# ChangwuLiu/InGVIO

Measured on AMD Instinct MI355X. Metric: ekf_updates_per_sec, higher is better.
Workload: dtype f64; 1 GPU; BASELINE configs[1]: synthetic stereo MSCKF, 150 feats x 11 clones, state dim N=249 (update at N), 512 independent filters per GPU; step = propagate(k=10)+clone+MSCKF update+marginalise; filters_per_gpu=512, feats=150, clones=11, state_dim=249, imu_steps=10, parallelism=independent filters, 1 rank(s), no data-path collective

## Files before the change

### include/ingvio_hip.h

```cpp
#ifndef INGVIO_HIP_H
#define INGVIO_HIP_H

#include <stddef.h>

#ifdef __cplusplus
extern "C" {
#endif

#define INGVIO_OK 0
#define INGVIO_NO_ROWS 1
#define INGVIO_NEG_DIAG 2
#define INGVIO_REJECTED 3
#define INGVIO_E_ARG (-1)
#define INGVIO_E_CAPACITY (-2)
#define INGVIO_E_HIP (-3)
#define INGVIO_E_NOT_IN_STATE (-4)
#define INGVIO_E_UNSUPPORTED (-5)
#define INGVIO_E_NOT_PD (-6)

typedef struct ingvio_ctx ingvio_ctx;

typedef struct {
    int batch;
    int n_max;
// ... 305 lines not shown
    int track;
    int anchor;
    double pf[3];
} ingvio_lm_init_cand;
typedef struct {
    int n_cand; const ingvio_lm_init_cand* cand;
    int n_drop; const int* drop_cols;
} ingvio_lm_init_block;
int ingvio_landmark_init_nominal(ingvio_ctx* ctx, int b0, int nb, const ingvio_lm_init_block* blocks, const ingvio_msckf_opts* opts,
                                 double chi2_mult, int do_chi2, int cand_cap,
                                 int* added, int* new_idx, int* slot, double* chi2, double* dx, int* status);
int ingvio_debug_landmark_init_rows(ingvio_ctx* ctx, int b, const ingvio_lm_init_cand* cand, const ingvio_msckf_opts* opts,
                                    int n_drop, const int* drop_cols, double* H_old, double* H_new, double* res, int* m_out);
int ingvio_frame_run(ingvio_ctx* ctx, int restore_prior);
int ingvio_set_frame_parts(ingvio_ctx* ctx, int parts);
int ingvio_frame_fetch(ingvio_ctx* ctx, int b0, int nb, double* dx_out, int* accepted, int* rows_out);
int ingvio_frame_fetch_begin(ingvio_ctx* ctx, int b0, int nb);
int ingvio_frame_fetch_end(ingvio_ctx* ctx, double* dx_out, int* accepted, int* rows_out);

int ingvio_debug_msckf_info(ingvio_ctx* ctx, int b, double* A_out, int* ncol_out);

int ingvio_debug_info_solution(ingvio_ctx* ctx, int b, double* out, int count);

int ingvio_debug_tracks_read(ingvio_ctx* ctx, int b, unsigned long long* mask, double* uv, double* pf);

int ingvio_debug_staged_frame(ingvio_ctx* ctx, int b, int* n_clones, int* n_feat, int* clone_idx, double* clone_R, double* clone_p,
                              int* anchor, int* dof, unsigned long long* obs_mask, double* pf, double* uv);

int ingvio_debug_read(ingvio_ctx* ctx, long long* out, int n);

// ... 10 lines not shown
```

### ingvio_amd/capi.py

```python
import ctypes as C
import os

import numpy as np

_HERE = os.path.dirname(os.path.abspath(__file__))
LIB_PATH = os.environ.get("INGVIO_HIP_LIB") or os.path.join(_HERE, "lib", "libingvio_hip.so")

c_dp = C.POINTER(C.c_double)
c_ip = C.POINTER(C.c_int)
c_up = C.POINTER(C.c_ulonglong)

OK, NO_ROWS, NEG_DIAG, REJECTED = 0, 1, 2, 3
E_ARG, E_CAPACITY, E_HIP, E_NOT_IN_STATE, E_UNSUPPORTED, E_NOT_PD = -1, -2, -3, -4, -5, -6
R_SCALAR, R_DIAG, R_FULL = 0, 1, 2

EXPORTS = [
    "ingvio_ctx_create", "ingvio_ctx_destroy", "ingvio_sync", "ingvio_ctx_stream", "ingvio_f_max", "ingvio_c_max", "ingvio_last_error", "ingvio_ldp",
    "ingvio_build_id",
    "ingvio_cov_set", "ingvio_cov_get", "ingvio_get_n", "ingvio_cov_get_marginal", "ingvio_cov_snapshot",
    "ingvio_cov_restore", "ingvio_propagate", "ingvio_propagate_fused", "ingvio_augment_clone", "ingvio_marginalize",
    "ingvio_append_independent", "ingvio_ekf_update", "ingvio_chi2_gamma", "ingvio_msckf_update", "ingvio_msckf_update_tri", "ingvio_qr_compress",
    "ingvio_frame_stage", "ingvio_frame_stage_async", "ingvio_frame_set_imu_noise", "ingvio_frame_fetch_begin", "ingvio_frame_fetch_end", "ingvio_tracks_create", "ingvio_frame_stage_tracks", "ingvio_frame_run", "ingvio_set_frame_parts", "ingvio_frame_fetch", "ingvio_profile_enable", "ingvio_profile_select",
    "ingvio_profile_reset",
    "ingvio_profile_get", "ingvio_set_msckf_method", "ingvio_set_qr_method", "ingvio_landmark_stage", "ingvio_landmark_run",
    "ingvio_landmark_fetch", "ingvio_frame_run_phase", "ingvio_info_set", "ingvio_debug_read", "ingvio_triangulate",
    "ingvio_gnss_front_stage", "ingvio_gnss_front_fetch", "ingvio_gnss_update_batch", "ingvio_gnss_stage", "ingvio_gnss_run", "ingvio_gnss_fetch", "ingvio_mld", "ingvio_debug_msckf_info", "ingvio_debug_info_solution",
    "ingvio_info_reduce", "ingvio_info_commit", "ingvio_gnss_sat_eval",
    "ingvio_chi2_gamma_multi", "ingvio_ekf_update_batch", "ingvio_add_variable_delayed_invertible", "ingvio_add_variable_delayed", "ingvio_add_variable_delayed_batch", "ingvio_replace_var_linear",
    "ingvio_nominal_create", "ingvio_nominal_set", "ingvio_nominal_get", "ingvio_nominal_box_plus", "ingvio_frame_stage_tracks_nominal",
    "ingvio_nominal_set_gnss", "ingvio_nominal_get_gnss", "ingvio_gnss_front_stage_nominal", "ingvio_landmark_stage_nominal",
    "ingvio_landmark_init_nominal", "ingvio_debug_landmark_init_rows", "ingvio_nominal_tail",
    "ingvio_debug_tracks_read", "ingvio_debug_staged_frame",
    "ingvio_gnss_frame_stage_nominal", "ingvio_debug_gnss_fused_last", "ingvio_debug_nominal_update_post",
]

NOM_NONE, NOM_SE23, NOM_SE3, NOM_VEC3, NOM_SCALAR, NOM_LANDMARK = -1, 0, 1, 2, 3, 4
NOM_VAL = 15
# ... 948 lines not shown
        fn = self.L.ingvio_frame_stage_async if use_async else self.L.ingvio_frame_stage

        def call(_keep=(keeps, chi2, sa, fa, o, sg)):
            self._chk(fn(self.h, b0, nb, sa, fa, C.byref(o), _d(sg), int(enable_gnss), C.c_double(sigma_cb), C.c_double(sigma_rw)))
        return call

    def frame_set_imu_noise(self, b0, noise):
        nz = f64(np.asarray(noise, dtype=np.float64).reshape(-1, 6))
        self._chk(self.L.ingvio_frame_set_imu_noise(self.h, int(b0), nz.shape[0], _d(nz)))

    def frame_run(self, restore_prior=False):
        self._chk(self.L.ingvio_frame_run(self.h, 1 if restore_prior else 0))

    def set_frame_parts(self, parts):
        self._chk(self.L.ingvio_set_frame_parts(self.h, int(parts)))

    def frame_fetch(self, b0=0, nb=None):
        nb = self.batch if nb is None else nb
        dx = np.zeros((nb, self.ldp)); acc = np.zeros((nb, self.f_max), dtype=np.int32); rows = np.zeros(nb, dtype=np.int32)
        self._chk(self.L.ingvio_frame_fetch(self.h, b0, nb, _d(dx), _i(acc), _i(rows)))
        return dx, acc, rows

    def frame_fetch_begin(self, b0=0, nb=None):
        nb = self.batch if nb is None else nb
        self._fetch_nb = nb
        self._chk(self.L.ingvio_frame_fetch_begin(self.h, b0, nb))

    def frame_fetch_end(self):
        nb = self._fetch_nb
        dx = np.empty((nb, self.ldp)); acc = np.empty((nb, self.f_max), dtype=np.int32); rows = np.empty(nb, dtype=np.int32)
# ... 85 lines not shown
```

### ingvio_amd/csrc/capi.hip

```cpp
#include "../../include/ingvio_hip.h"
#include "dev_common.h"
#include "launch_ekf.h"
#include "launch_msckf.h"
#include "launch_factored.h"
#include "launch_tri.h"
#include "launch_tracks.h"
#include "launch_lm.h"
#include "launch_delayed.h"
#include "launch_qr.h"
#include "launch_chol.h"
#include "launch_gnss.h"
#include "launch_lmbatch.h"
#include "launch_nominal.h"
#include "launch_tail.h"

#include <stdio.h>
#include <stdlib.h>
#include <string.h>
#include <unistd.h>
#include <string>
#include <atomic>
#include <cmath>
#include <condition_variable>
#include <functional>
// ... 125 lines not shown
    hipStream_t st2 = nullptr;
    hipEvent_t ev_fork = nullptr, ev_join = nullptr, ev_ref = nullptr;
    hipEvent_t ev_fetch = nullptr;
    int fetch_b0 = 0, fetch_nb = 0;
    hipStream_t st_copy = nullptr;
    hipEvent_t ev_copy = nullptr, ev_free[2] = { nullptr, nullptr };
    bool copy_pending = false, free_valid[2] = { false, false };
    int set_id = 0;
    struct PinSlab { char* p = nullptr; size_t cap = 0; hipEvent_t ev = nullptr; bool busy = false; };
    PinSlab pin[4];
    int pin_next = 0;
    struct PartStream { hipStream_t st = nullptr; hipEvent_t ev_gate = nullptr, ev_apply = nullptr, ev_done = nullptr; };
    PartStream part[4];
    int parts_alloc = 0;
    int parts_req = -1;
    bool split_pending = false;
    hipEvent_t tok_last = nullptr;
    hipEvent_t ev_split_fork = nullptr;
    hipStream_t run_st = nullptr;
    hipEvent_t tok_wait = nullptr, tok_rec = nullptr;
    struct Tracks { double *uv = nullptr, *pf = nullptr; unsigned long long* mask = nullptr; int t_max = 0; char* stage[2] = { nullptr, nullptr }; size_t stage_cap = 0; } trk;
    struct Nominal {
        int vmax = 0, ir = 0, dr = 0;
        int* ih = nullptr; double* dv = nullptr;
        int* ih_snap = nullptr; double* dv_snap = nullptr;
        double* dx = nullptr;
        std::vector<int> h_ih, h_ih_snap;
        bool has_snap = false;
        bool pending = false;
        bool frame = false;
// ... 555 lines not shown
    if (g.strong) { E.chi2 = g.chi2; E.chi2_len = g.chi2_len; E.gate_max_rows = 14; }
    RowsGateIn in{ g.H + (size_t)b0 * hs, g.res + (size_t)b0 * mld, g.noise + (size_t)b0 * mld, g.m + b0, g.colmap + (size_t)b0 * GNSS_NCW,
                   g.nc + b0, (int)hs, GNSS_NCW };
    {
        ProfScope p(c, PF_ROWGATE);
        if (launch_rows_gate(E, in, g.thr1, g.gamma + (size_t)b0 * mld, g.keep + (size_t)b0 * mld, c->run_st)) return INGVIO_E_CAPACITY;
    }
    { ProfScope p(c, PF_EKF_CORE); launch_ekf_core(E, c->run_st); }
    L.gY = E.Y; L.gYstride = ws; L.gm = g.mf + b0;
    g.fused_last = true; g.folded_last = true;
    g.results = true;
    return 0;
}

int run_msckf_factored(ingvio_ctx* c, int b0, int nb, const MsckfOpts& op, int stereo, int fmax_used,
                       const int* marg_idx = nullptr, int marg_size = 0, int phase = 0, bool gnss_fuse = false)
{
    FactoredLaunch L;
    memset(&L, 0, sizeof L);
    L.stereo = stereo; L.cv = view(c); L.fv = fview(c); L.op = op; L.b0 = b0; L.nb = nb;
    L.fmax_used = fmax_used > 0 ? fmax_used : 1;
    L.ncol_cap = 6 * c->d.c_max;
    for (int i = 0; i < nb; ++i) if (c->h_nclones[b0 + i] > L.c_used) L.c_used = c->h_nclones[b0 + i];
    L.gamma = c->d_gamma; L.accept = c->d_accept; L.used = c->d_used; L.rec = c->d_rec;
    L.Apart = c->d_Rpart + (size_t)b0 * c->G * c->rstride; L.chunk_used = c->d_chunk_used + (size_t)b0 * c->G;
    L.G = c->G; L.rstride = c->rstride; L.noise = c->d_noise + b0;
    L.Tflat = c->d_Tflat; L.tfstride = (size_t)c->ldp * 100; L.flat_nb = std::min(c->d.batch, APPLY_FLAT_NB);
    L.Asum = c->d_Asum ? c->d_Asum + (size_t)b0 * c->rstride : nullptr; L.used_sum = c->d_used_sum ? c->d_used_sum + b0 : nullptr;
#ifdef INGVIO_ALT_KERNELS
    static const bool few_off = [] { const char* e = getenv("INGVIO_FEW"); return e && !strcmp(e, "off"); }();
    if (few_off) { L.Tflat = nullptr; L.Asum = nullptr; }
// ... 16 lines not shown
    if (phase != 2) {
        if (c->tok_wait) HIPCHK(c, hipStreamWaitEvent(c->run_st, c->tok_wait, 0));
        {
            const bool pon = c->prof && (c->prof_only < 0 || c->prof_only == PF_GATE2);
            int used = 0;
            if (pon) { hipEventCreate(&L.prof_a); hipEventCreate(&L.prof_b); L.prof_used = &used; }
            L.stage = 0;
            const int grc = launch_factored(L, c->run_st);
            if (pon) {
                if (used) c->recs.push_back({ PF_GATE2, L.prof_a, L.prof_b });
                else { hipEventDestroy(L.prof_a); hipEventDestroy(L.prof_b); }
                L.prof_a = nullptr; L.prof_b = nullptr; L.prof_used = nullptr;
            }
            if (grc) return INGVIO_E_UNSUPPORTED;
        }
        { ProfScope p(c, PF_GRAM); L.stage = 1; launch_factored(L, c->run_st); }
        if (c->tok_rec) HIPCHK(c, hipEventRecord(c->tok_rec, c->run_st));
    }
    if (forked) {
        HIPCHK(c, hipStreamWaitEvent(c->st2, c->ev_fork, 0));
        L.stage = 6; launch_factored(L, c->st2);
        HIPCHK(c, hipEventRecord(c->ev_ref, c->st2));
        L.stage = 7; launch_factored(L, c->st2);
        HIPCHK(c, hipEventRecord(c->ev_join, c->st2));
    }
    if (phase == 1) return last_launch(c);
    if (forked) {
        ProfScope p(c, PF_INFO);
        HIPCHK(c, hipStreamWaitEvent(c->run_st, c->ev_ref, 0));
        L.stage = 8; launch_factored(L, c->run_st);
        HIPCHK(c, hipStreamWaitEvent(c->run_st, c->ev_join, 0));
        L.stage = 9; launch_factored(L, c->run_st);
    } else {
        if (big) { ProfScope p(c, PF_INFO); L.stage = 5; launch_factored(L, c->run_st); }
        { ProfScope p(c, PF_INFO); L.stage = 2; launch_factored(L, c->run_st); }
    }
    if (gnss_fuse) { if (int rc = gnss_in_frame_launch(c, b0, nb, L)) return rc; }
    if (phase == 2 && c->tok_wait) HIPCHK(c, hipStreamWaitEvent(c->run_st, c->tok_wait, 0));
    { ProfScope p(c, PF_APPLY); L.stage = 3; launch_factored(L, c->run_st); }
    if (phase == 2 && c->tok_rec) HIPCHK(c, hipEventRecord(c->tok_rec, c->run_st));
    return last_launch(c);
}

int run_msckf(ingvio_ctx* c, int b0, int nb, const MsckfOpts& op, int stereo, int fmax_used)
{
    if (c->method == 1) return run_msckf_factored(c, b0, nb, op, stereo, fmax_used);
    MsckfLaunch L;
    memset(&L, 0, sizeof L);
    L.stereo = stereo; L.cv = view(c); L.fv = fview(c); L.op = op; L.b0 = b0; L.nb = nb;
    L.fmax_used = fmax_used > 0 ? fmax_used : 1;
    L.gamma = c->d_gamma; L.accept = c->d_accept; L.used = c->d_used;
    L.Rpart = c->d_Rpart + (size_t)b0 * c->G * c->rstride; L.chunk_used = c->d_chunk_used + (size_t)b0 * c->G;
    L.G = c->G; L.rstride = c->rstride;
    L.Hout = c->d_H + (size_t)b0 * c->hstride; L.res_out = c->d_res + (size_t)b0 * c->mld;
    L.colmap = c->d_colmap + (size_t)b0 * c->cstride; L.m_out = c->d_m + b0; L.nc_out = c->d_nc + b0;
    L.mld = c->mld; L.hstride = c->hstride; L.cstride = c->cstride;
    { ProfScope p(c, PF_GATE); L.stage = 0; if (launch_msckf(L, c->st)) return INGVIO_E_UNSUPPORTED; }
    { ProfScope p(c, PF_FOLD); L.stage = 1; launch_msckf(L, c->st); }
    { ProfScope p(c, PF_MERGE); L.stage = 2; launch_msckf(L, c->st); }
    EkfLaunch E;
    memset(&E, 0, sizeof E);
// ... 135 lines not shown
    if (desc->c_max > bigwin_cmax()) return INGVIO_E_CAPACITY;
    if (desc->m_max > 128) return INGVIO_E_CAPACITY;
    int ndev = 0;
    if (hipGetDeviceCount(&ndev) != hipSuccess || ndev <= desc->device) return INGVIO_E_HIP;
    ingvio_ctx* c = new ingvio_ctx();
    c->d = *desc;
    if (c->d.m_max < 1) c->d.m_max = 32;
    c->err.clear();
    if (hipSetDevice(desc->device) != hipSuccess) { delete c; return INGVIO_E_HIP; }
    c->own_stream = desc->stream == nullptr;
    if (c->own_stream) {
        if (hipStreamCreateWithFlags(&c->st, hipStreamNonBlocking) != hipSuccess) { delete c; return INGVIO_E_HIP; }
    } else c->st = (hipStream_t)desc->stream;
    c->run_st = c->st;
    if (const char* e = getenv("INGVIO_FRAME_PARTS")) c->parts_req = atoi(e);
    if (desc->c_max > 16) {
        int lo = 0, hi = 0;
        hipDeviceGetStreamPriorityRange(&lo, &hi);
        if (hipStreamCreateWithPriority(&c->st2, hipStreamNonBlocking, hi) != hipSuccess) c->st2 = nullptr;
        if (c->st2 && (hipEventCreateWithFlags(&c->ev_fork, hipEventDisableTiming) != hipSuccess ||
                       hipEventCreateWithFlags(&c->ev_ref, hipEventDisableTiming) != hipSuccess ||
                       hipEventCreateWithFlags(&c->ev_join, hipEventDisableTiming) != hipSuccess)) { hipStreamDestroy(c->st2); c->st2 = nullptr; }
    }
    const int B = desc->batch;
    c->ldp = (desc->n_max + 15) & ~15;
    const int cls0 = desc->c_max > 16 ? bigwin_cmax() : msckf_cmax_class(desc->c_max);
    const int cpad = cls0 > desc->c_max ? cls0 : desc->c_max;
    const int mcap = c->d.m_max > 6 * cpad ? c->d.m_max : 6 * cpad;
    c->mld = (mcap + 15) & ~15;
    c->nc_cap = c->ldp > mcap ? c->ldp : mcap;
// ... 2859 lines not shown
    if (wait_inputs(c)) return INGVIO_E_HIP;
    launch_restore_propagate(c, restore_prior, strips_valid(c, restore_prior), 0, B, c->st);
    mirror_restore_clone(c, restore_prior);
    const bool with_lm = lm_in_frame(c);
    const bool fuse = c->method == 1 && !with_lm;
    const bool lm_oop = with_lm && c->method == 1;
    const bool gnss_here = gnss_in_frame(c), gnss_fuse = fuse && gnss_folds(c);
    const bool gnss_nomf = c->gn.staged && c->gn.frame_nom;
    if (gnss_nomf) {
        auto& g = c->gn;
        HIPCHK(c, hipMemsetAsync(g.dxf, 0, 8 * (size_t)B * c->ldp, c->st));
        HIPCHK(c, hipMemsetAsync(g.stf, 0, sizeof(int) * (size_t)B, c->st));
        HIPCHK(c, hipMemsetAsync(g.mf, 0, sizeof(int) * (size_t)B, c->st));
        g.own_status = true; g.results = true; g.fused_last = true; g.folded_last = false;
    }
    int rc = fuse     ? run_msckf_factored(c, 0, B, c->st_op, c->st_stereo, c->st_fmax_used, c->d_idx, 6, 0, gnss_fuse)
             : lm_oop ? run_msckf_factored(c, 0, B, c->st_op, c->st_stereo, c->st_fmax_used, c->d_zero_idx, 0)
                      : run_msckf(c, 0, B, c->st_op, c->st_stereo, c->st_fmax_used);
    if (rc) return rc;
    if (lm_oop) {
        if (!c->apply_flipped) launch_post_marg(view(c), 0, B, c->d_zero_idx, 0, c->st);
        for (int b = 0; b < B; ++b) c->h_cur[b] ^= 1;
    }
    const bool lm_nom = with_lm && c->lm.nominal;
    if (lm_nom) landmark_gather_launch(c, c->d_dx, 0, B);
    bool lm_fused = false;
    if (with_lm) { rc = landmark_update_launch(c, 0, B, c->d_idx, 6, &lm_fused); if (rc) return rc; }
    if (!(fuse && c->apply_flipped)) {
        ProfScope p(c, PF_MARG);
        if (fuse || lm_fused) launch_post_marg(view(c), 0, B, c->d_idx, 6, c->st);
        else launch_marginalize(view(c), 0, B, c->d.n_max, c->d_idx, 6, c->st);
    }
// ... 63 lines not shown
    const int P = std::min(c->parts_req > 0 ? c->parts_req : 1, 4);
    const bool gnss_fuse = gnss_folds(c);
    if (P > 1 && c->method == 1 && !lm_in_frame(c) && c->d.c_max <= 16 && (!gnss_in_frame(c) || gnss_fuse) && B >= 16 * P)
        return frame_run_split(c, restore_prior, P, gnss_fuse);
    return frame_run_whole(c, restore_prior);
}

int ingvio_frame_run(ingvio_ctx* c, int restore_prior) { return frame_run_impl(c, restore_prior, 0); }
int ingvio_set_frame_parts(ingvio_ctx* c, int parts)
{
    if (!c || parts < -1 || parts > 4) return INGVIO_E_ARG;
    ENTER(c);
    c->parts_req = parts == 0 ? 1 : parts;
    return INGVIO_OK;
}
int ingvio_frame_run_phase(ingvio_ctx* c, int restore_prior, int phase)
{
    if (phase < 0 || phase > 2) return INGVIO_E_ARG;
    return frame_run_impl(c, restore_prior, phase);
}

int ingvio_info_set(ingvio_ctx* c, int b, const double* A, int ncol, int n_accepted)
{
    ENTER(c);
    if (check_range(c, b, 1) || !A || ncol < 6 || (size_t)ncol * (ncol + 1) > (size_t)c->rstride || n_accepted < 0) return INGVIO_E_ARG;
    std::vector<int> used(c->G, 0);
    used[0] = n_accepted;
    int rc = up(c, c->d_Rpart + (size_t)b * c->G * c->rstride, A, 8 * (size_t)ncol * (ncol + 1));
    rc |= up(c, c->d_chunk_used + (size_t)b * c->G, used.data(), sizeof(int) * (size_t)c->G);
    if (rc) return INGVIO_E_HIP;
// ... 87 lines not shown
    return last_launch(c);
}

int ingvio_set_msckf_method(ingvio_ctx* c, int method)
{
    ENTER(c);
    if (!c || method < 0 || method > 1) return INGVIO_E_ARG;
    c->method = method;
    return INGVIO_OK;
}

int ingvio_debug_msckf_info(ingvio_ctx* c, int b, double* A_out, int* ncol_out)
{
    ENTER(c);
    if (check_range(c, b, 1) || !A_out || !ncol_out) return INGVIO_E_ARG;
    int C = 0;
    if (down_sync(c, &C, c->d_nclones + b, sizeof(int))) return INGVIO_E_HIP;
    const int ncol = 6 * C;
    *ncol_out = ncol;
    const size_t w = (size_t)ncol + 1;
    for (size_t e = 0; e < (size_t)ncol * w; ++e) A_out[e] = 0.0;
    if (c->method == 1) {
        std::vector<int> used(c->G);
        if (down_sync(c, used.data(), c->d_chunk_used + (size_t)b * c->G, sizeof(int) * (size_t)c->G)) return INGVIO_E_HIP;
        std::vector<double> part((size_t)ncol * w);
        for (int g = 0; g < c->G; ++g) {
            if (!used[g]) continue;
            if (down_sync(c, part.data(), c->d_Rpart + ((size_t)b * c->G + g) * c->rstride, 8 * part.size())) return INGVIO_E_HIP;
            for (size_t e = 0; e < part.size(); ++e) A_out[e] += part[e];
        }
// ... 139 lines not shown
```

### ingvio_amd/csrc/kernels_factored.hip

```cpp
#include <algorithm>
#include <stdlib.h>
#include <string.h>
#include "launch_factored.h"

#include "gate_kernel.h"
#include "gate5_kernel.h"
#include "gate5m_kernel.h"

#define GATE_FPW 1
template <int CMAX, bool STEREO>
__global__ __launch_bounds__(GATE_FPW * WAVE) __attribute__((amdgpu_waves_per_eu(2, 4))) void k_feat_gate3(
    CovView cv, FrameView fv, MsckfOpts op, int b0, int nb, int fmax_used, double* __restrict__ gamma_out,
    int* __restrict__ accept_out, double* __restrict__ rec_out)
{
    gate3_body<CMAX, STEREO, GATE_FPW, false>(cv, fv, op, b0, nb, fmax_used, gamma_out, accept_out, rec_out);
}

#ifndef GATE4_WPE
#define GATE4_WPE 2
#endif
#ifndef GATE4_WPE_MAX
#define GATE4_WPE_MAX 6
#endif
template <int CMAX>
// ... 21 lines not shown
}

#define GRAM_NB 8
#define GRAM_NT 256
#ifndef GRAM2_ZFORM
#define GRAM2_ZFORM 1
#endif
__device__ __forceinline__ double gram_rsqrt(double x)
{
    double y = __builtin_amdgcn_rsq(x);
    double e = fma(-x * y, y, 1.0);
    y = fma(y * e, fma(e, 0.375, 0.5), y);
    e = fma(-x * y, y, 1.0);
    return fma(y * e, 0.5, y);
}
template <int CMAX>
struct Gram2Cfg {
    static constexpr int NC = 6 * CMAX;
    static constexpr int TI = (NC + 15) / 16;
    static constexpr int TJ = (NC + 1 + 15) / 16;
    static constexpr int LDW = 16 * TJ;
    static constexpr int NTILE = TI * TJ;
    static constexpr int NUP = TI * TJ - TI * (TI - 1) / 2;
    static constexpr int TPW = (NUP + 3) / 4;
    static constexpr int KR = 3 * GRAM_NB;
    static constexpr int SPW = 34;
};
template <int CMAX>
struct Gram2Batch {
    using Cfg = Gram2Cfg<CMAX>;
    double Bm[Cfg::KR][Cfg::LDW];
    double Ym[Cfg::KR][Cfg::LDW];
    double sp[CMAX * CMAX <= 128 ? 2 : 1][GRAM_NB][CMAX][Cfg::SPW];
};
template <int CMAX>
struct Gram2Out {
    using Cfg = Gram2Cfg<CMAX>;
    double A2[Cfg::NC][Cfg::NC + 2];
    double S[CMAX][CMAX][34];
};

template <int CMAX, bool STEREO>
__global__ __launch_bounds__(GRAM_NT, 2) void k_feat_gram2(
    FrameView fv, MsckfOpts op, int b0, const int* __restrict__ accept_in, int* __restrict__ used_out,
    double* __restrict__ Apart, int* __restrict__ chunk_used, int G, int rstride)
{
    using Cfg = Gram2Cfg<CMAX>;
    constexpr int NC = Cfg::NC, TJ = Cfg::TJ, LDW = Cfg::LDW, NTILE = Cfg::NTILE, TPW = Cfg::TPW, KR = Cfg::KR;
    constexpr int NUP = Cfg::NUP, TI = Cfg::TI, RPO = STEREO ? 4 : 2;
    extern __shared__ __attribute__((aligned(16))) char smem_raw[];
    Gram2Batch<CMAX>& sb = *reinterpret_cast<Gram2Batch<CMAX>*>(smem_raw);
    Gram2Out<CMAX>& so = *reinterpret_cast<Gram2Out<CMAX>*>(smem_raw);
    constexpr size_t UNI = sizeof(Gram2Batch<CMAX>) > sizeof(Gram2Out<CMAX>) ? sizeof(Gram2Batch<CMAX>) : sizeof(Gram2Out<CMAX>);
    int* sUse = reinterpret_cast<int*>(smem_raw + ((UNI + 15) / 16) * 16);
    int* sList = sUse + fv.fmax;
    __shared__ int sNu;
    __shared__ double sPose[16][12];
    const int bl = blockIdx.y, b = b0 + bl, g = blockIdx.x, tid = threadIdx.x, lane = tid & 63, wave = __builtin_amdgcn_readfirstlane(tid >> 6);
    const int F = fv.n_feat[b], C = fv.n_clones[b], ncol = 6 * C;
    for (int e = tid; e < 12 * C; e += GRAM_NT) {
        const int c = e / 12, q = e - 12 * c;
        sPose[c][q] = q < 9 ? fv.clone_R[((size_t)b * fv.cmax + c) * 9 + q] : fv.clone_p[((size_t)b * fv.cmax + c) * 3 + q - 9];
    }

    dbg_stamp(32);
    for (int j = tid; j < F; j += GRAM_NT) {
        int use = accept_in[(size_t)b * fv.fmax + j];
        if (use && op.max_accept > 0) {
            int rank = 0;
            for (int q = 0; q < j; ++q) rank += accept_in[(size_t)b * fv.fmax + q];
            if (rank >= op.max_accept) use = 0;
        }
        sUse[j] = use;
        if (g == 0) used_out[(size_t)b * fv.fmax + j] = use;
    }
    for (int e = tid; e < KR * LDW; e += GRAM_NT) { (&sb.Bm[0][0])[e] = 0.0; (&sb.Ym[0][0])[e] = 0.0; }
    __syncthreads();
    if (wave == 0) {
        int cnt = 0;
        for (int base = 0; base < F; base += WAVE) {
            const int j = base + lane;
            const bool u = j < F && sUse[j];
            const unsigned long long m = __ballot(u);
            if (u) sList[cnt + __popcll(m & ((1ULL << lane) - 1ULL))] = j;
            cnt += __popcll(m);
        }
        if (lane == 0) sNu = cnt;
    }
    __syncthreads();
    const int nu = sNu, per = (nu + G - 1) / G;
    const int q0 = g * per, q1 = min(nu, q0 + per);

    dbg_stamp(33);
    int tiA[TPW], tjA[TPW];
#pragma unroll
    for (int u = 0; u < TPW; ++u) {
        int t = wave + 4 * u, ti = 0;
        while (ti < TI - 1 && t >= TJ - ti) { t -= TJ - ti; ++ti; }
        tiA[u] = ti; tjA[u] = ti + t;
    }
    double4_f acc[TPW];
#pragma unroll
    for (int u = 0; u < TPW; ++u) acc[u] = double4_f{ 0.0, 0.0, 0.0, 0.0 };
    constexpr bool OVL = CMAX * CMAX <= 128;
    const int ptid = OVL ? tid - 128 : tid;
    const int pc = ptid >= 0 ? ptid / CMAX : 0, pa = ptid >= 0 ? ptid - pc * CMAX : 0;
    const bool pairlane = ptid >= 0 && ptid < CMAX * CMAX;
    double sS1[9], sNX[9], sS3[9], s4[3], s5[3];
#pragma unroll
    for (int i = 0; i < 9; ++i) { sS1[i] = 0.0; sNX[i] = 0.0; sS3[i] = 0.0; }
#pragma unroll
    for (int i = 0; i < 3; ++i) { s4[i] = 0.0; s5[i] = 0.0; }
// ... 36 lines not shown
        }
    };
    auto sum16 = [](double v) {
#ifdef GRAM_SHFL_SUM
        v += __shfl_xor(v, 8, 16); v += __shfl_xor(v, 4, 16); v += __shfl_xor(v, 2, 16); v += __shfl_xor(v, 1, 16);
#else
        v += row_ror_f64<8>(v); v += row_ror_f64<4>(v); v += row_ror_f64<2>(v); v += row_ror_f64<1>(v);
#endif
        return v;
    };
    fetch(q0);
    auto do_p2 = [&](int qb, int buf, int nthr, bool rows, bool sparse) {
        const int nbf = min(GRAM_NB, q1 - qb);
        dbg_stamp(34);
        if (rows && nbf < GRAM_NB) {
            for (int e = tid; e < (KR - 3 * nbf) * LDW; e += nthr) { (&sb.Bm[3 * nbf][0])[e] = 0.0; (&sb.Ym[3 * nbf][0])[e] = 0.0; }
        }
        dbg_stamp(35);
        if (ft < nbf * 16) {
            const int f = ft >> 4, c = ft & 15;
            const int a = in_anchor;
            const double px = in_pf[0], py = in_pf[1], pz = in_pf[2];
            bool obs = c < C && ((in_mask >> c) & 1ULL);
            double N[9], h[3];
#pragma unroll
            for (int i = 0; i < 9; ++i) N[i] = 0.0;
#pragma unroll
            for (int i = 0; i < 3; ++i) h[i] = 0.0;
            if (obs) {
                double Gm[RPO][3], rs[RPO];
                obs = feat_obs<STEREO>(sPose[c], sPose[c] + 9, in_uv, px, py, pz, op, Gm, rs);
// ... 38 lines not shown
                double Bt[9], Bp[9];
#pragma unroll
                for (int i = 0; i < 9; ++i) { Bt[i] = cn * NX[i]; Bp[i] = -pl * N[i]; }
                if (c == a) {
                    double T[9];
                    mulX(Nsa, px, py, pz, T);
#pragma unroll
                    for (int i = 0; i < 9; ++i) Bt[i] = -T[i];
                }
#if GRAM2_ZFORM
                const double s0 = Ns[0] > 0.0 ? gram_rsqrt(Ns[0]) : 0.0, r0 = s0 * s0;
                const double l10 = Ns[1] * r0, l20 = Ns[2] * r0;
                const double d1 = Ns[4] - l10 * Ns[1], s1 = d1 > 0.0 ? gram_rsqrt(d1) : 0.0, r1 = s1 * s1;
                const double t21 = Ns[5] - l20 * Ns[1], l21 = t21 * r1;
                const double d2 = (Ns[8] - l20 * Ns[2]) - l21 * t21, s2 = d2 > 0.0 ? gram_rsqrt(d2) : 0.0;
#pragma unroll
                for (int q = 0; q < 3; ++q) {
                    {
                        const double y0 = Bt[q], y1 = Bt[3 + q] - l10 * y0, y2 = (Bt[6 + q] - l20 * y0) - l21 * y1;
                        sb.Bm[3 * f + 0][6 * c + q] = s0 * y0; sb.Bm[3 * f + 1][6 * c + q] = s1 * y1; sb.Bm[3 * f + 2][6 * c + q] = s2 * y2;
                    }
                    {
                        const double y0 = Bp[q], y1 = Bp[3 + q] - l10 * y0, y2 = (Bp[6 + q] - l20 * y0) - l21 * y1;
                        sb.Bm[3 * f + 0][6 * c + 3 + q] = s0 * y0; sb.Bm[3 * f + 1][6 * c + 3 + q] = s1 * y1; sb.Bm[3 * f + 2][6 * c + 3 + q] = s2 * y2;
                    }
                }
                if (c == 0) {
                    const double y0 = hs[0], y1 = hs[1] - l10 * y0, y2 = (hs[2] - l20 * y0) - l21 * y1;
                    sb.Bm[3 * f + 0][NC] = s0 * y0; sb.Bm[3 * f + 1][NC] = s1 * y1; sb.Bm[3 * f + 2][NC] = s2 * y2;
                }
#else
                double Nsi[9];
                inv3sym(Ns, Nsi);
                double Yt[9], Yp[9];
                mul33(Nsi, Bt, Yt);
                mul33(Nsi, Bp, Yp);
#pragma unroll
                for (int k = 0; k < 3; ++k)
#pragma unroll
                    for (int q = 0; q < 3; ++q) {
                        sb.Bm[3 * f + k][6 * c + q] = Bt[3 * k + q];
                        sb.Bm[3 * f + k][6 * c + 3 + q] = Bp[3 * k + q];
                        sb.Ym[3 * f + k][6 * c + q] = Yt[3 * k + q];
                        sb.Ym[3 * f + k][6 * c + 3 + q] = Yp[3 * k + q];
                    }
                if (c == 0) {
#pragma unroll
                    for (int k = 0; k < 3; ++k) sb.Bm[3 * f + k][NC] = hs[k];
                }
#endif
              }
              if (sparse) {
                double* sp = sb.sp[buf][f][c < CMAX ? c : 0];
                double S1[9];
                mulXt(NX, px, py, pz, S1);
#pragma unroll
                for (int i = 0; i < 9; ++i) { sp[i] = cn * S1[i]; sp[9 + i] = cn * pl * NX[i]; }
                sp[18] = cn * (pz * h[1] - py * h[2]);
                sp[19] = cn * (px * h[2] - pz * h[0]);
                sp[20] = cn * (py * h[0] - px * h[1]);
// ... 2 lines not shown
#pragma unroll
                for (int i = 0; i < 3; ++i) sp[30 + i] = pl * h[i];
                sp[33] = (obs || c == 0) ? (double)a : -1.0;
              }
            }
        }
    };
    auto do_p3a = [&](int qb) {
        const int nbf = min(GRAM_NB, q1 - qb);
        const int nst = (3 * nbf + 3) >> 2;
#pragma unroll
        for (int st = 0; st < KR / 4; ++st) {
            if (st < nst) {
#pragma unroll
                for (int u = 0; u < TPW; ++u) {
                    if (wave + 4 * u < NUP) {
                        const int ti = tiA[u], tj = tjA[u];
                        const double af = (GRAM2_ZFORM ? sb.Bm : sb.Ym)[4 * st + kq][16 * ti + l15];
                        const double bf = sb.Bm[4 * st + kq][16 * tj + l15];
                        acc[u] = __builtin_amdgcn_mfma_f64_16x16x4f64(af, bf, acc[u], 0, 0, 0);
                    }
                }
            }
        }
    };
    auto do_p3b = [&](int qb, int buf) {
        const int nbf = min(GRAM_NB, q1 - qb);
        if (P3U) {
            if (ulane) {
#pragma unroll
                for (int f = 0; f < GRAM_NB; ++f) {
                    if (f < nbf) {
                        const double* sp = sb.sp[buf][f][uc];
// ... 44 lines not shown
        }
    } else {
        for (int qb = q0; qb < q1; qb += GRAM_NB) {
            do_p2(qb, 0, GRAM_NT, true, true);
            lds_barrier();
            fetch(qb + GRAM_NB);
            do_p3a(qb);
            do_p3b(qb, 0);
            lds_barrier();
        }
    }

    dbg_stamp(39);
#pragma unroll
    for (int u = 0; u < TPW; ++u) {
        if (wave + 4 * u < NUP) {
            const int ti = tiA[u], tj = tjA[u];
            const int jc = 16 * tj + l15;
#pragma unroll
            for (int r = 0; r < 4; ++r) {
                const int i = 16 * ti + kq + 4 * r;
                if (i < NC && jc <= NC) so.A2[i][jc] = acc[u][r];
            }
        }
    }
    if (P3U) {
        if (ulane) {
#pragma unroll
            for (int a2 = 0; a2 < CMAX; ++a2)
#pragma unroll
                for (int i = 0; i < 3; ++i) {
                    const int v = 3 * uj + i;
                    so.S[uc][a2][v < 18 ? v : (v < 21 ? v + 9 : (v < 30 ? v - 3 : v))] = sacc[3 * a2 + i];
                }
        }
    } else if (pairlane) {
        double* S = so.S[pc][pa];
#pragma unroll
        for (int i = 0; i < 9; ++i) { S[i] = sS1[i]; S[9 + i] = sNX[i]; S[18 + i] = sS3[i]; }
#pragma unroll
        for (int i = 0; i < 3; ++i) { S[27 + i] = s4[i]; S[30 + i] = s5[i]; }
    }
    __syncthreads();
    double* out = Apart + ((size_t)bl * G + g) * rstride;
    if (pairlane && pc < C && pa < C) {
        const int c = pc, c2 = pa;
        double blk[36];
#pragma unroll
        for (int i = 0; i < 36; ++i) blk[i] = 0.0;
        double bb[6] = { 0.0, 0.0, 0.0, 0.0, 0.0, 0.0 };
        if (c == c2) {
            for (int a = 0; a < C; ++a) {
                const double* S = so.S[c][a];
                const double* Sa = so.S[a][c];
#pragma unroll
                for (int q = 0; q < 3; ++q)
#pragma unroll
                    for (int q2 = 0; q2 < 3; ++q2) {
                        blk[6 * q + q2] += S[3 * q + q2] + Sa[3 * q + q2];
                        blk[6 * q + 3 + q2] -= S[9 + 3 * q2 + q];
// ... 725 lines not shown
    const int midx = marg_idx ? marg_idx[bl] : -1;
    double d;
    if (midx >= 0 && r >= midx && r < midx + msize) {
        d = 0.0;
        for (int k = 0; k < MP; ++k) d += Pc[r + (size_t)k * ld] * tvec[k];
    } else {
        double p[4] = { 0.0, 0.0, 0.0, 0.0 };
        for (int k4 = 0; k4 < MP / 4; ++k4)
#pragma unroll
            for (int q = 0; q < 4; ++q) p[q] += Pc[r + (size_t)(4 * k4 + q) * ld] * tvec[4 * k4 + q];
        d = (p[0] + p[1]) + (p[2] + p[3]);
    }
    dx_all[(size_t)b * ld + r] = d;
}

template <int CMAX, bool STEREO>
static void launch_ft(const FactoredLaunch& L, hipStream_t st)
{
    if (L.stage == 0) {
        const int nb8 = (L.nb + 7) / 8 * 8;
#ifdef INGVIO_ALT_KERNELS
        static const bool gate3 = [] { const char* e = getenv("INGVIO_GATE"); return e && e[0] == '3'; }();
#else
        constexpr bool gate3 = false;
#endif
        static const bool gate4 = [] { const char* e = getenv("INGVIO_GATE"); return e && e[0] == '4'; }();
        if constexpr (STEREO && CMAX <= 11) {
            if (!gate3 && !gate4) {
                LAUNCH_GATE(L, (k_feat_gate5<CMAX>), dim3(nb8 * ((L.fmax_used + 3) / 4)), dim3(WAVE), 0, st, L.cv, L.fv, L.op, L.b0, L.nb, L.fmax_used,
                                   L.gamma, L.accept);
                return;
            }
// ... 24 lines not shown
            static const bool gram3 = [] { const char* e = getenv("INGVIO_GRAM"); return e && e[0] == '3'; }();
            if (gram3) {
                constexpr size_t uni3 = sizeof(Gram3Batch<CMAX>) > sizeof(Gram2Out<CMAX>) ? sizeof(Gram3Batch<CMAX>) : sizeof(Gram2Out<CMAX>);
                const size_t sm3 = ((uni3 + 15) / 16) * 16 + 2 * sizeof(int) * (size_t)L.fv.fmax;
                static size_t attr_sm3 = 0;
                if (sm3 > attr_sm3) {
                    hipFuncSetAttribute((const void*)k_feat_gram3<CMAX, STEREO>, hipFuncAttributeMaxDynamicSharedMemorySize, (int)sm3);
                    attr_sm3 = sm3;
                }
                hipLaunchKernelGGL((k_feat_gram3<CMAX, STEREO>), dim3(L.G, L.nb), dim3(GRAM_NT), sm3, st,
                                   L.fv, L.op, L.b0, L.accept, L.used, L.Apart, L.chunk_used, L.G, L.rstride);
                return;
            }
        }
#endif
        constexpr size_t uni = sizeof(Gram2Batch<CMAX>) > sizeof(Gram2Out<CMAX>) ? sizeof(Gram2Batch<CMAX>) : sizeof(Gram2Out<CMAX>);
        const size_t sm = ((uni + 15) / 16) * 16 + 2 * sizeof(int) * (size_t)L.fv.fmax;
        static size_t attr_sm = 0;
        if (sm > attr_sm) {
            hipFuncSetAttribute((const void*)k_feat_gram2<CMAX, STEREO>, hipFuncAttributeMaxDynamicSharedMemorySize, (int)sm);
            attr_sm = sm;
        }
        hipLaunchKernelGGL((k_feat_gram2<CMAX, STEREO>), dim3(L.G, L.nb), dim3(GRAM_NT), sm, st,
                           L.fv, L.op, L.b0, L.accept, L.used, L.Apart, L.chunk_used, L.G, L.rstride);
    }
}

__global__ __launch_bounds__(256) void k_chunk_sum(const double* __restrict__ Apart, const int* __restrict__ chunk_used, int G, int rstride,
                                                   double* __restrict__ out, int* __restrict__ used_out)
{
    const int bl = blockIdx.y, e = blockIdx.x * 256 + threadIdx.x;
    const int* cu = chunk_used + (size_t)bl * G;
    const double* A = Apart + (size_t)bl * G * rstride;
    unsigned long long mask = 0;
    int total = 0;
    for (int g = 0; g < G; ++g) { mask |= (cu[g] != 0 ? 1ull : 0ull) << g; total += cu[g]; }
    if (e < rstride) {
        double s = 0.0;
#pragma unroll 8
// ... 81 lines not shown
#define INFO_DISPATCH(NC)                                                                                                   \
        {                                                                                                                   \
            const size_t sm = sizeof(double) * (size_t)NC * (2 * NC + 1) + sizeof(int) * (size_t)NC + 16;                     \
            hipFuncSetAttribute((const void*)k_info_update<NC>, hipFuncAttributeMaxDynamicSharedMemorySize, (int)sm);         \
            hipLaunchKernelGGL(k_info_update<NC>, dim3(L.nb), dim3(INFO_NT), sm, st, L.cv, L.fv, L.b0, L.Apart, L.chunk_used, \
                               L.G, L.rstride, L.noise, L.T, L.mstride, L.Pc, L.ystride, L.dx, L.m_out, L.nc_out, L.status,  \
                               L.marg_idx, L.pc_base);                                                                      \
        }
        if (ncm <= 36) { INFO_DISPATCH(36) } else if (ncm <= 66) { INFO_DISPATCH(66) } else if (ncm <= 72) { INFO_DISPATCH(72) } else { INFO_DISPATCH(96) }
#undef INFO_DISPATCH
        return 0;
    }
    const int cm = cm_sel;
    const int cls = cm <= 6 ? 6 : (cm <= 11 ? 11 : (cm <= 12 ? 12 : (cm <= 16 ? 16 : -1)));
    if (cls < 0) return -1;
#define DISPATCH(CM)                                                         \
    if (cls == CM) { if (L.stereo) launch_ft<CM, true>(L, st); else launch_ft<CM, false>(L, st); return 0; }
    DISPATCH(6)
    DISPATCH(11)
    DISPATCH(12)
    DISPATCH(16)
#undef DISPATCH
    return -1;
}

int dbg_read_factored(long long* out, int n) { return dbg_read_local(out, n); }
```

### ingvio_amd/csrc/launch_factored.h

```cpp
#pragma once
#include "dev_common.h"

#ifndef INGVIO_APPLY_FLAT_NB
#define INGVIO_APPLY_FLAT_NB 64
#endif
constexpr int APPLY_FLAT_NB = INGVIO_APPLY_FLAT_NB;

struct FactoredLaunch {
    int stage;
    int stereo;
    CovView cv;
    FrameView fv;
    MsckfOpts op;
    int b0, nb, fmax_used;
    double* gamma;
    int* accept;
    int* used;
    double* rec;
    double* Apart;
    double* Asum;
    int* used_sum;
    double* Tflat;
    size_t tfstride;
    int flat_nb;
// ... 1 lines not shown
    int G, rstride;
    const double* noise;
    double* T;
    int mstride, n_cap;
    double* Pc;
    int ystride;
    double* dx;
    int* m_out;
    int* nc_out;
    int* status;
    const int* marg_idx;
    int marg_size;
    int* pc_base;
    int* flip_cnt;
    int* did_flip;
    double* big_sg;
    double* big_wk;
    int ncol_cap;
    int c_used;
    const int* gcolmap;
    const int* gnc;
    int gcstride;
    double* gW;
    size_t gWstride;
    const double* gY;
    size_t gYstride;
    const int* gm;
    hipEvent_t prof_a, prof_b;
    int* prof_used;
};
// ... 21 lines not shown
```

Before: 1.067 million updates/s.

## Form reduced Gram matrix without reference clone columns in frame-step MSCKF

Adds a reduced Gram variant that drops the last (reference) clone's six columns when forming the factored MSCKF normal equations during the frame step. This shrinks the per-feature MFMA Gram tiles and LDS footprint for C≤12 clones, relying on the downstream info solve gauging out that clone. It also reorders wave-to-tile assignment in the reduced path and removes the unused Y buffer in Z-form builds. It is on by default, with a runtime switch and an environment override, and the debug readback of the full [A|b] is disabled when the reduced form was used.

```diff
diff --git a/include/ingvio_hip.h b/include/ingvio_hip.h
--- a/include/ingvio_hip.h
+++ b/include/ingvio_hip.h
@@ -343,6 +343,7 @@
                                     int n_drop, const int* drop_cols, double* H_old, double* H_new, double* res, int* m_out);
 int ingvio_frame_run(ingvio_ctx* ctx, int restore_prior);
 int ingvio_set_frame_parts(ingvio_ctx* ctx, int parts);
+int ingvio_set_gram_reduced(ingvio_ctx* ctx, int on);
 int ingvio_frame_fetch(ingvio_ctx* ctx, int b0, int nb, double* dx_out, int* accepted, int* rows_out);
 int ingvio_frame_fetch_begin(ingvio_ctx* ctx, int b0, int nb);
 int ingvio_frame_fetch_end(ingvio_ctx* ctx, double* dx_out, int* accepted, int* rows_out);
diff --git a/ingvio_amd/capi.py b/ingvio_amd/capi.py
--- a/ingvio_amd/capi.py
+++ b/ingvio_amd/capi.py
@@ -20,7 +20,7 @@
     "ingvio_cov_set", "ingvio_cov_get", "ingvio_get_n", "ingvio_cov_get_marginal", "ingvio_cov_snapshot",
     "ingvio_cov_restore", "ingvio_propagate", "ingvio_propagate_fused", "ingvio_augment_clone", "ingvio_marginalize",
     "ingvio_append_independent", "ingvio_ekf_update", "ingvio_chi2_gamma", "ingvio_msckf_update", "ingvio_msckf_update_tri", "ingvio_qr_compress",
-    "ingvio_frame_stage", "ingvio_frame_stage_async", "ingvio_frame_set_imu_noise", "ingvio_frame_fetch_begin", "ingvio_frame_fetch_end", "ingvio_tracks_create", "ingvio_frame_stage_tracks", "ingvio_frame_run", "ingvio_set_frame_parts", "ingvio_frame_fetch", "ingvio_profile_enable", "ingvio_profile_select",
+    "ingvio_frame_stage", "ingvio_frame_stage_async", "ingvio_frame_set_imu_noise", "ingvio_frame_fetch_begin", "ingvio_frame_fetch_end", "ingvio_tracks_create", "ingvio_frame_stage_tracks", "ingvio_frame_run", "ingvio_set_frame_parts", "ingvio_set_gram_reduced", "ingvio_frame_fetch", "ingvio_profile_enable", "ingvio_profile_select",
     "ingvio_profile_reset",
     "ingvio_profile_get", "ingvio_set_msckf_method", "ingvio_set_qr_method", "ingvio_landmark_stage", "ingvio_landmark_run",
     "ingvio_landmark_fetch", "ingvio_frame_run_phase", "ingvio_info_set", "ingvio_debug_read", "ingvio_triangulate",
@@ -999,6 +999,9 @@
 
     def set_frame_parts(self, parts):
         self._chk(self.L.ingvio_set_frame_parts(self.h, int(parts)))
+
+    def set_gram_reduced(self, on):
+        self._chk(self.L.ingvio_set_gram_reduced(self.h, 1 if on else 0))
 
     def frame_fetch(self, b0=0, nb=None):
         nb = self.batch if nb is None else nb
diff --git a/ingvio_amd/csrc/capi.hip b/ingvio_amd/csrc/capi.hip
--- a/ingvio_amd/csrc/capi.hip
+++ b/ingvio_amd/csrc/capi.hip
@@ -163,6 +163,8 @@
     PartStream part[4];
     int parts_alloc = 0;
     int parts_req = -1;
+    int gram_reduced = 1;
+    int gram_red_last = 0;
     bool split_pending = false;
     hipEvent_t tok_last = nullptr;
     hipEvent_t ev_split_fork = nullptr;
@@ -748,7 +750,7 @@
 }
 
 int run_msckf_factored(ingvio_ctx* c, int b0, int nb, const MsckfOpts& op, int stereo, int fmax_used,
-                       const int* marg_idx = nullptr, int marg_size = 0, int phase = 0, bool gnss_fuse = false)
+                       const int* marg_idx = nullptr, int marg_size = 0, int phase = 0, bool gnss_fuse = false, bool frame_step = false)
 {
     FactoredLaunch L;
     memset(&L, 0, sizeof L);
@@ -795,7 +797,10 @@
             }
             if (grc) return INGVIO_E_UNSUPPORTED;
         }
+        c->gram_red_last = 0;
+        L.gram_red = frame_step && phase == 0 && c->gram_reduced; L.gram_was_red = &c->gram_red_last;
         { ProfScope p(c, PF_GRAM); L.stage = 1; launch_factored(L, c->run_st); }
+        L.gram_was_red = nullptr;
         if (c->tok_rec) HIPCHK(c, hipEventRecord(c->tok_rec, c->run_st));
     }
     if (forked) {
@@ -826,6 +831,7 @@
 int run_msckf(ingvio_ctx* c, int b0, int nb, const MsckfOpts& op, int stereo, int fmax_used)
 {
     if (c->method == 1) return run_msckf_factored(c, b0, nb, op, stereo, fmax_used);
+    c->gram_red_last = 0;
     MsckfLaunch L;
     memset(&L, 0, sizeof L);
     L.stereo = stereo; L.cv = view(c); L.fv = fview(c); L.op = op; L.b0 = b0; L.nb = nb;
@@ -991,6 +997,7 @@
     } else c->st = (hipStream_t)desc->stream;
     c->run_st = c->st;
     if (const char* e = getenv("INGVIO_FRAME_PARTS")) c->parts_req = atoi(e);
+    if (const char* e = getenv("INGVIO_GRAM_REDUCED")) c->gram_reduced = atoi(e) != 0;
     if (desc->c_max > 16) {
         int lo = 0, hi = 0;
         hipDeviceGetStreamPriorityRange(&lo, &hi);
@@ -3880,8 +3887,8 @@
         HIPCHK(c, hipMemsetAsync(g.mf, 0, sizeof(int) * (size_t)B, c->st));
         g.own_status = true; g.results = true; g.fused_last = true; g.folded_last = false;
     }
-    int rc = fuse     ? run_msckf_factored(c, 0, B, c->st_op, c->st_stereo, c->st_fmax_used, c->d_idx, 6, 0, gnss_fuse)
-             : lm_oop ? run_msckf_factored(c, 0, B, c->st_op, c->st_stereo, c->st_fmax_used, c->d_zero_idx, 0)
+    int rc = fuse     ? run_msckf_factored(c, 0, B, c->st_op, c->st_stereo, c->st_fmax_used, c->d_idx, 6, 0, gnss_fuse, true)
+             : lm_oop ? run_msckf_factored(c, 0, B, c->st_op, c->st_stereo, c->st_fmax_used, c->d_zero_idx, 0, 0, false, true)
                       : run_msckf(c, 0, B, c->st_op, c->st_stereo, c->st_fmax_used);
     if (rc) return rc;
     if (lm_oop) {
@@ -3975,6 +3982,13 @@
     c->parts_req = parts == 0 ? 1 : parts;
     return INGVIO_OK;
 }
+int ingvio_set_gram_reduced(ingvio_ctx* c, int on)
+{
+    if (!c) return INGVIO_E_ARG;
+    ENTER(c);
+    c->gram_reduced = on ? 1 : 0;
+    return INGVIO_OK;
+}
 int ingvio_frame_run_phase(ingvio_ctx* c, int restore_prior, int phase)
 {
     if (phase < 0 || phase > 2) return INGVIO_E_ARG;
@@ -4092,6 +4106,10 @@
 {
     ENTER(c);
     if (check_range(c, b, 1) || !A_out || !ncol_out) return INGVIO_E_ARG;
+    if (c->method == 1 && c->gram_red_last) {
+        c->err = "the last frame step formed [A | b] in reduced form; run it with ingvio_set_gram_reduced(ctx, 0) to read the full [A | b]";
+        return INGVIO_E_UNSUPPORTED;
+    }
     int C = 0;
     if (down_sync(c, &C, c->d_nclones + b, sizeof(int))) return INGVIO_E_HIP;
     const int ncol = 6 * C;
diff --git a/ingvio_amd/csrc/kernels_factored.hip b/ingvio_amd/csrc/kernels_factored.hip
--- a/ingvio_amd/csrc/kernels_factored.hip
+++ b/ingvio_amd/csrc/kernels_factored.hip
@@ -59,9 +59,9 @@
     e = fma(-x * y, y, 1.0);
     return fma(y * e, 0.5, y);
 }
-template <int CMAX>
+template <int CMAX, bool RED = false>
 struct Gram2Cfg {
-    static constexpr int NC = 6 * CMAX;
+    static constexpr int NC = RED ? 6 * (CMAX - 1) : 6 * CMAX;
     static constexpr int TI = (NC + 15) / 16;
     static constexpr int TJ = (NC + 1 + 15) / 16;
     static constexpr int LDW = 16 * TJ;
@@ -71,38 +71,45 @@
     static constexpr int KR = 3 * GRAM_NB;
     static constexpr int SPW = 34;
 };
-template <int CMAX>
+template <int CMAX, bool RED = false>
 struct Gram2Batch {
-    using Cfg = Gram2Cfg<CMAX>;
+    using Cfg = Gram2Cfg<CMAX, RED>;
     double Bm[Cfg::KR][Cfg::LDW];
+#if !GRAM2_ZFORM
     double Ym[Cfg::KR][Cfg::LDW];
+#endif
     double sp[CMAX * CMAX <= 128 ? 2 : 1][GRAM_NB][CMAX][Cfg::SPW];
 };
-template <int CMAX>
+template <int CMAX, bool RED = false>
 struct Gram2Out {
-    using Cfg = Gram2Cfg<CMAX>;
+    using Cfg = Gram2Cfg<CMAX, RED>;
     double A2[Cfg::NC][Cfg::NC + 2];
     double S[CMAX][CMAX][34];
 };
-
-template <int CMAX, bool STEREO>
+template <int CMAX, bool RED = false>
+constexpr size_t gram2_lds_bytes()
+{
+    return ((std::max(sizeof(Gram2Batch<CMAX, RED>), sizeof(Gram2Out<CMAX, RED>)) + 15) / 16) * 16;
+}
+
+template <int CMAX, bool STEREO, bool RED = false>
 __global__ __launch_bounds__(GRAM_NT, 2) void k_feat_gram2(
     FrameView fv, MsckfOpts op, int b0, const int* __restrict__ accept_in, int* __restrict__ used_out,
     double* __restrict__ Apart, int* __restrict__ chunk_used, int G, int rstride)
 {
-    using Cfg = Gram2Cfg<CMAX>;
+    using Cfg = Gram2Cfg<CMAX, RED>;
     constexpr int NC = Cfg::NC, TJ = Cfg::TJ, LDW = Cfg::LDW, NTILE = Cfg::NTILE, TPW = Cfg::TPW, KR = Cfg::KR;
     constexpr int NUP = Cfg::NUP, TI = Cfg::TI, RPO = STEREO ? 4 : 2;
     extern __shared__ __attribute__((aligned(16))) char smem_raw[];
-    Gram2Batch<CMAX>& sb = *reinterpret_cast<Gram2Batch<CMAX>*>(smem_raw);
-    Gram2Out<CMAX>& so = *reinterpret_cast<Gram2Out<CMAX>*>(smem_raw);
-    constexpr size_t UNI = sizeof(Gram2Batch<CMAX>) > sizeof(Gram2Out<CMAX>) ? sizeof(Gram2Batch<CMAX>) : sizeof(Gram2Out<CMAX>);
-    int* sUse = reinterpret_cast<int*>(smem_raw + ((UNI + 15) / 16) * 16);
+    Gram2Batch<CMAX, RED>& sb = *reinterpret_cast<Gram2Batch<CMAX, RED>*>(smem_raw);
+    Gram2Out<CMAX, RED>& so = *reinterpret_cast<Gram2Out<CMAX, RED>*>(smem_raw);
+    int* sUse = reinterpret_cast<int*>(smem_raw + gram2_lds_bytes<CMAX, RED>());
     int* sList = sUse + fv.fmax;
     __shared__ int sNu;
     __shared__ double sPose[16][12];
     const int bl = blockIdx.y, b = b0 + bl, g = blockIdx.x, tid = threadIdx.x, lane = tid & 63, wave = __builtin_amdgcn_readfirstlane(tid >> 6);
     const int F = fv.n_feat[b], C = fv.n_clones[b], ncol = 6 * C;
+    const int cref = RED ? C - 1 : -1;
     for (int e = tid; e < 12 * C; e += GRAM_NT) {
         const int c = e / 12, q = e - 12 * c;
         sPose[c][q] = q < 9 ? fv.clone_R[((size_t)b * fv.cmax + c) * 9 + q] : fv.clone_p[((size_t)b * fv.cmax + c) * 3 + q - 9];
@@ -119,7 +126,12 @@
         sUse[j] = use;
         if (g == 0) used_out[(size_t)b * fv.fmax + j] = use;
     }
-    for (int e = tid; e < KR * LDW; e += GRAM_NT) { (&sb.Bm[0][0])[e] = 0.0; (&sb.Ym[0][0])[e] = 0.0; }
+    for (int e = tid; e < KR * LDW; e += GRAM_NT) {
+        (&sb.Bm[0][0])[e] = 0.0;
+#if !GRAM2_ZFORM
+        (&sb.Ym[0][0])[e] = 0.0;
+#endif
+    }
     __syncthreads();
     if (wave == 0) {
         int cnt = 0;
@@ -137,10 +149,14 @@
     const int q0 = g * per, q1 = min(nu, q0 + per);
 
     dbg_stamp(33);
+#ifndef GRAM2_RED_DEAL
+#define GRAM2_RED_DEAL 1
+#endif
+    const int wdeal = (RED && GRAM2_RED_DEAL) ? (wave ^ 2) : wave;
     int tiA[TPW], tjA[TPW];
 #pragma unroll
     for (int u = 0; u < TPW; ++u) {
-        int t = wave + 4 * u, ti = 0;
+        int t = wdeal + 4 * u, ti = 0;
         while (ti < TI - 1 && t >= TJ - ti) { t -= TJ - ti; ++ti; }
         tiA[u] = ti; tjA[u] = ti + t;
     }
@@ -207,7 +223,12 @@
         const int nbf = min(GRAM_NB, q1 - qb);
         dbg_stamp(34);
         if (rows && nbf < GRAM_NB) {
-            for (int e = tid; e < (KR - 3 * nbf) * LDW; e += nthr) { (&sb.Bm[3 * nbf][0])[e] = 0.0; (&sb.Ym[3 * nbf][0])[e] = 0.0; }
+            for (int e = tid; e < (KR - 3 * nbf) * LDW; e += nthr) {
+                (&sb.Bm[3 * nbf][0])[e] = 0.0;
+#if !GRAM2_ZFORM
+                (&sb.Ym[3 * nbf][0])[e] = 0.0;
+#endif
+            }
         }
         dbg_stamp(35);
         if (ft < nbf * 16) {
@@ -276,15 +297,17 @@
                 const double d1 = Ns[4] - l10 * Ns[1], s1 = d1 > 0.0 ? gram_rsqrt(d1) : 0.0, r1 = s1 * s1;
                 const double t21 = Ns[5] - l20 * Ns[1], l21 = t21 * r1;
                 const double d2 = (Ns[8] - l20 * Ns[2]) - l21 * t21, s2 = d2 > 0.0 ? gram_rsqrt(d2) : 0.0;
-#pragma unroll
-                for (int q = 0; q < 3; ++q) {
-                    {
-                        const double y0 = Bt[q], y1 = Bt[3 + q] - l10 * y0, y2 = (Bt[6 + q] - l20 * y0) - l21 * y1;
-                        sb.Bm[3 * f + 0][6 * c + q] = s0 * y0; sb.Bm[3 * f + 1][6 * c + q] = s1 * y1; sb.Bm[3 * f + 2][6 * c + q] = s2 * y2;
-                    }
-                    {
-                        const double y0 = Bp[q], y1 = Bp[3 + q] - l10 * y0, y2 = (Bp[6 + q] - l20 * y0) - l21 * y1;
-                        sb.Bm[3 * f + 0][6 * c + 3 + q] = s0 * y0; sb.Bm[3 * f + 1][6 * c + 3 + q] = s1 * y1; sb.Bm[3 * f + 2][6 * c + 3 + q] = s2 * y2;
+                if (!RED || c != cref) {
+#pragma unroll
+                    for (int q = 0; q < 3; ++q) {
+                        {
+                            const double y0 = Bt[q], y1 = Bt[3 + q] - l10 * y0, y2 = (Bt[6 + q] - l20 * y0) - l21 * y1;
+                            sb.Bm[3 * f + 0][6 * c + q] = s0 * y0; sb.Bm[3 * f + 1][6 * c + q] = s1 * y1; sb.Bm[3 * f + 2][6 * c + q] = s2 * y2;
+                        }
+                        {
+                            const double y0 = Bp[q], y1 = Bp[3 + q] - l10 * y0, y2 = (Bp[6 + q] - l20 * y0) - l21 * y1;
+                            sb.Bm[3 * f + 0][6 * c + 3 + q] = s0 * y0; sb.Bm[3 * f + 1][6 * c + 3 + q] = s1 * y1; sb.Bm[3 * f + 2][6 * c + 3 + q] = s2 * y2;
+                        }
                     }
                 }
                 if (c == 0) {
@@ -297,15 +320,17 @@
                 double Yt[9], Yp[9];
                 mul33(Nsi, Bt, Yt);
                 mul33(Nsi, Bp, Yp);
-#pragma unroll
-                for (int k = 0; k < 3; ++k)
-#pragma unroll
-                    for (int q = 0; q < 3; ++q) {
-                        sb.Bm[3 * f + k][6 * c + q] = Bt[3 * k + q];
-                        sb.Bm[3 * f + k][6 * c + 3 + q] = Bp[3 * k + q];
-                        sb.Ym[3 * f + k][6 * c + q] = Yt[3 * k + q];
-                        sb.Ym[3 * f + k][6 * c + 3 + q] = Yp[3 * k + q];
-                    }
+                if (!RED || c != cref) {
+#pragma unroll
+                    for (int k = 0; k < 3; ++k)
+#pragma unroll
+                        for (int q = 0; q < 3; ++q) {
+                            sb.Bm[3 * f + k][6 * c + q] = Bt[3 * k + q];
+                            sb.Bm[3 * f + k][6 * c + 3 + q] = Bp[3 * k + q];
+                            sb.Ym[3 * f + k][6 * c + q] = Yt[3 * k + q];
+                            sb.Ym[3 * f + k][6 * c + 3 + q] = Yp[3 * k + q];
+                        }
+                }
                 if (c == 0) {
 #pragma unroll
                     for (int k = 0; k < 3; ++k) sb.Bm[3 * f + k][NC] = hs[k];
@@ -338,9 +363,13 @@
             if (st < nst) {
 #pragma unroll
                 for (int u = 0; u < TPW; ++u) {
-                    if (wave + 4 * u < NUP) {
+                    if (wdeal + 4 * u < NUP) {
                         const int ti = tiA[u], tj = tjA[u];
-                        const double af = (GRAM2_ZFORM ? sb.Bm : sb.Ym)[4 * st + kq][16 * ti + l15];
+#if GRAM2_ZFORM
+                        const double af = sb.Bm[4 * st + kq][16 * ti + l15];
+#else
+                        const double af = sb.Ym[4 * st + kq][16 * ti + l15];
+#endif
                         const double bf = sb.Bm[4 * st + kq][16 * tj + l15];
                         acc[u] = __builtin_amdgcn_mfma_f64_16x16x4f64(af, bf, acc[u], 0, 0, 0);
                     }
@@ -415,7 +444,7 @@
     dbg_stamp(39);
 #pragma unroll
     for (int u = 0; u < TPW; ++u) {
-        if (wave + 4 * u < NUP) {
+        if (wdeal + 4 * u < NUP) {
             const int ti = tiA[u], tj = tjA[u];
             const int jc = 16 * tj + l15;
 #pragma unroll
@@ -444,7 +473,7 @@
     }
     __syncthreads();
     double* out = Apart + ((size_t)bl * G + g) * rstride;
-    if (pairlane && pc < C && pa < C) {
+    if (pairlane && pc < C && pa < C && pc != cref && pa != cref) {
         const int c = pc, c2 = pa;
         double blk[36];
 #pragma unroll
@@ -1200,8 +1229,22 @@
     dx_all[(size_t)b * ld + r] = d;
 }
 
+template <int CMAX, bool STEREO, bool RED>
+static void launch_gram2(const FactoredLaunch& L, hipStream_t st)
+{
+    const size_t sm = gram2_lds_bytes<CMAX, RED>() + 2 * sizeof(int) * (size_t)L.fv.fmax;
+    static size_t attr_sm = 0;
+    if (sm > attr_sm) {
+        hipFuncSetAttribute((const void*)k_feat_gram2<CMAX, STEREO, RED>, hipFuncAttributeMaxDynamicSharedMemorySize, (int)sm);
+        attr_sm = sm;
+    }
+    hipLaunchKernelGGL((k_feat_gram2<CMAX, STEREO, RED>), dim3(L.G, L.nb), dim3(GRAM_NT), sm, st,
+                       L.fv, L.op, L.b0, L.accept, L.used, L.Apart, L.chunk_used, L.G, L.rstride);
+    if (L.gram_was_red) *L.gram_was_red = RED ? 1 : 0;
+}
+
 template <int CMAX, bool STEREO>
-static void launch_ft(const FactoredLaunch& L, hipStream_t st)
+static void launch_ft(const FactoredLaunch& L, hipStream_t st, bool gram_red)
 {
     if (L.stage == 0) {
         const int nb8 = (L.nb + 7) / 8 * 8;
@@ -1256,15 +1299,10 @@
             }
         }
 #endif
-        constexpr size_t uni = sizeof(Gram2Batch<CMAX>) > sizeof(Gram2Out<CMAX>) ? sizeof(Gram2Batch<CMAX>) : sizeof(Gram2Out<CMAX>);
-        const size_t sm = ((uni + 15) / 16) * 16 + 2 * sizeof(int) * (size_t)L.fv.fmax;
-        static size_t attr_sm = 0;
-        if (sm > attr_sm) {
-            hipFuncSetAttribute((const void*)k_feat_gram2<CMAX, STEREO>, hipFuncAttributeMaxDynamicSharedMemorySize, (int)sm);
-            attr_sm = sm;
-        }
-        hipLaunchKernelGGL((k_feat_gram2<CMAX, STEREO>), dim3(L.G, L.nb), dim3(GRAM_NT), sm, st,
-                           L.fv, L.op, L.b0, L.accept, L.used, L.Apart, L.chunk_used, L.G, L.rstride);
+        if constexpr (CMAX <= 12) {
+            if (gram_red) { launch_gram2<CMAX, STEREO, true>(L, st); return; }
+        }
+        launch_gram2<CMAX, STEREO, false>(L, st);
     }
 }
 
@@ -1376,8 +1414,17 @@
     const int cm = cm_sel;
     const int cls = cm <= 6 ? 6 : (cm <= 11 ? 11 : (cm <= 12 ? 12 : (cm <= 16 ? 16 : -1)));
     if (cls < 0) return -1;
+#ifdef INGVIO_ALT_KERNELS
+    static const bool full_solve = [] {
+        const char* e = getenv("INGVIO_INFO_GAUGE"); const char* s = getenv("INGVIO_INFO_SOLVE");
+        return (e && !strcmp(e, "off")) || (s && !strcmp(s, "gj"));
+    }();
+#else
+    constexpr bool full_solve = false;
+#endif
+    const bool gram_red = L.stage == 1 && L.gram_red && !L.op.selected_variant && cls <= 12 && !full_solve;
 #define DISPATCH(CM)                                                         \
-    if (cls == CM) { if (L.stereo) launch_ft<CM, true>(L, st); else launch_ft<CM, false>(L, st); return 0; }
+    if (cls == CM) { if (L.stereo) launch_ft<CM, true>(L, st, gram_red); else launch_ft<CM, false>(L, st, gram_red); return 0; }
     DISPATCH(6)
     DISPATCH(11)
     DISPATCH(12)
diff --git a/ingvio_amd/csrc/launch_factored.h b/ingvio_amd/csrc/launch_factored.h
--- a/ingvio_amd/csrc/launch_factored.h
+++ b/ingvio_amd/csrc/launch_factored.h
@@ -39,6 +39,8 @@
     int* pc_base;
     int* flip_cnt;
     int* did_flip;
+    int gram_red;
+    int* gram_was_red;
     double* big_sg;
     double* big_wk;
     int ncol_cap;
```

New measurement: 1.089 million updates/s, median of 6. +2.0%, better.
